# rkin100g/Nerf-Replication

Hardware: AMD Instinct MI355X
Metric: rays/sec (800x800, 64+128 samples) (higher is better)
Workload: dtype f32; 1 GPU; lego-shaped 800x800 frame = 640000 pinhole rays, 64 coarse + 128 fine hierarchical samples, 8+1-layer W=256 NeRF x2, seeded synthetic weights (latest.pth unavailable offline); BASELINE.json configs[1]; parallelism=ray-tile shard x1 (each rank generates and renders only its tile) + 1 all_gather

## Files before the change

nerf_replication_amd/_lib.py:

```python
import ctypes
import os
import subprocess

import torch

_HERE = os.path.dirname(os.path.abspath(__file__))
LIB_PATH = os.path.join(_HERE, "libnerf_mi355x.so")
CSRC = os.path.join(_HERE, "csrc")

N_SAMPLES = 64
N_IMPORTANCE = 128
PREC_F32 = 0
PREC_F16 = 1
PREC_F32X = 2
PREC_F16S = 3
PRECISIONS = {"f32": PREC_F32, "fp32": PREC_F32, "f16": PREC_F16S, "fp16": PREC_F16S, "f16s": PREC_F16S, "f16m32": PREC_F16, "f32x": PREC_F32X}


def fp32_accurate(precision_name: str) -> bool:
    return PRECISIONS[precision_name] in (PREC_F32, PREC_F32X)


_TABLE = """
nerf_abi_version  i32 :
# ... 87 lines not shown


def _protos(signatures):
    return {name: (_RETURN[ret], [_ctype(k) for k in kinds]) for name, (ret, kinds) in signatures.items()}


_PROTOS = _protos(SIGNATURES)

_TABLE_NN = """
nerf_nn_abi_version  i32 :
nerf_fused_mlp_save_floats  i64 : i64 i32 i32
nerf_fused_mlp_grad_floats  i64 : i64 i32 i32 i32
nerf_fused_mlp_forward  status : f32* i64 i32 i32 i32 i32 i32 f32*[] f32*[] f32* f32* stream
nerf_fused_mlp_backward  status : f32* f32* f32* i64 i32 i32 i32 i32 i32 f32*[] f32* f32* f32*[] f32*[] f32* stream
nerf_sh4_encode  status : f32* i64 f32* stream
nerf_field_points  status : f32* f32* f32* i64 i64 i32 i32* i64 f32[3] f32[3] f32 f32* stream
nerf_field_color_inputs  status : f32* f32* i32* i64 i64 i32 f32* f32* stream
nerf_field_color_inputs_backward  status : f32* f32* i64 f32* stream
nerf_field_raw_scatter  status : f32* f32* i32* i64 i64 f32* stream
nerf_field_raw_gather  status : f32* i32* i64 i64 f32* f32* stream
"""
NN_SIGNATURES = _parse_table(_TABLE_NN)
NN_EXPORTS = tuple(NN_SIGNATURES)
_NN_PROTOS = _protos(NN_SIGNATURES)

_TABLE_FIELD = """
nerf_field_density_seed  status : f32* i64 i64 i32 f32* stream
nerf_field_points_backward  status : f32* f32* f32* i64 i64 i32 i32* i64 f32[3] f32[3] f32 f32* f32* i32 f32* f32* f32* stream
nerf_field_sh_gradient  status : f32* i32* i64 i64 i32 f32* stream
nerf_sh4_encode_backward  status : f32* f32* i64 f32* stream
"""
FIELD_SIGNATURES = _parse_table(_TABLE_FIELD)
FIELD_EXPORTS = tuple(FIELD_SIGNATURES)
_FIELD_PROTOS = _protos(FIELD_SIGNATURES)

_TABLE_HASHGRID = """
nerf_hashgrid_deterministic_workspace_bytes  i64 : i64 i32
nerf_hashgrid_deterministic_guard_bits  i32 : i64 i32
nerf_hashgrid_backward_deterministic  status : f32* f32* i64 i32 i32 i32 i32[] f32[] f32* void* i64 stream
"""
HASHGRID_SIGNATURES = _parse_table(_TABLE_HASHGRID)
HASHGRID_EXPORTS = tuple(HASHGRID_SIGNATURES)
_HASHGRID_PROTOS = _protos(HASHGRID_SIGNATURES)

_TABLE_NN_EXACT = """
nerf_fused_mlp_exact_workspace_bytes  i64 : i32 i32 i32 i32
nerf_fused_mlp_exact_guard_bits  i32 : i64
nerf_fused_mlp_backward_exact  status : f32* f32* f32* i64 i32 i32 i32 i32 i32 f32*[] f32* f32* f32*[] f32*[] f32* void* i64 stream
"""
NN_EXACT_SIGNATURES = _parse_table(_TABLE_NN_EXACT)
NN_EXACT_EXPORTS = tuple(NN_EXACT_SIGNATURES)
_NN_EXACT_PROTOS = _protos(NN_EXACT_SIGNATURES)

_lib = None


class NerfLibraryError(RuntimeError):
    pass


def build(verbose: bool = False) -> str:
    res = subprocess.run(["make", "-C", CSRC], capture_output=True, text=True)
    if res.returncode != 0:
        raise NerfLibraryError("building libnerf_mi355x.so failed:\n" + res.stdout + res.stderr)
    if verbose:
        print(res.stdout)
    return LIB_PATH


def load():
    global _lib
    if _lib is None:
        if not os.path.exists(LIB_PATH):
            raise NerfLibraryError(
                f"{LIB_PATH} is missing: build it with `make -C {CSRC}` (or __graft_entry__.build()); "
                "there is no CPU fallback for the render path")
        lib = ctypes.CDLL(LIB_PATH)
        for name, (res, args) in (list(_PROTOS.items()) + list(_NN_PROTOS.items()) + list(_FIELD_PROTOS.items()) +
                                  list(_HASHGRID_PROTOS.items()) + list(_NN_EXACT_PROTOS.items())):
            fn = getattr(lib, name)
            fn.restype, fn.argtypes = res, args
        if lib.nerf_abi_version() != 3:
            raise NerfLibraryError("libnerf_mi355x.so ABI version mismatch")
        if lib.nerf_nn_abi_version() != 1:
            raise NerfLibraryError("libnerf_mi355x.so small-network ABI version mismatch (include/nerf_mi355x_nn.h)")
        if lib.nerf_build_flags() != 0:
            raise NerfLibraryError(f"{LIB_PATH} is a timing build (nerf_build_flags() = {lib.nerf_build_flags()}): kernels "
                                   "compiled with NERF_*_HACK_* switches compute wrong results; rebuild with `make -C csrc`")
        _lib = lib
    return _lib


class strided:

    def __init__(self, tensor):
        self.tensor = tensor


def call(name, *args):
    for table in (SIGNATURES, NN_SIGNATURES, FIELD_SIGNATURES, HASHGRID_SIGNATURES, NN_EXACT_SIGNATURES):
        if name in table:
            break
    ret, kinds = table[name]
    has_stream = kinds[-1:] == ("stream",)
    if len(args) != len(kinds) - has_stream:
        raise TypeError(f"{name} takes {len(kinds) - has_stream} arguments ({len(args)} given)")
    dev = None

    def device_pointer(t, dtype, i):
        nonlocal dev
        if t is None:
            return None
        dense = not isinstance(t, strided)
        if not dense:
            t = t.tensor
        if not t.is_cuda:
            raise NerfLibraryError(f"{name}, argument {i}: the HIP render path needs tensors on a GPU (cuda) device; got a CPU tensor")
        if (dtype is not None and t.dtype != dtype) or (dense and not t.is_contiguous()):
            raise NerfLibraryError(f"{name}, argument {i}: expected a contiguous {dtype or 'byte'} tensor, got {t.dtype} with "
                                   f"strides {tuple(t.stride())}")
        if dev is None:
            dev = t.device
        elif t.device != dev:
            raise NerfLibraryError(f"{name}, argument {i}: a tensor on {t.device}, the earlier ones on {dev}")
        return t.data_ptr()

    cargs = []
    for i, (kind, a) in enumerate(zip(kinds, args)):
        if kind in _DTYPE:
            a = device_pointer(a, _DTYPE[kind], i)
        elif kind not in _SCALAR and a is not None:
            elem, _, length = kind[:-1].partition("[")
            if length and len(a) != int(length):
                raise NerfLibraryError(f"{name}, argument {i}: a host array of {length} is needed, got {len(a)}")
            if elem in _DTYPE:
                a = (ctypes.c_void_p * len(a))(*[device_pointer(t, _DTYPE[elem], i) for t in a])
            elif not isinstance(a, ctypes.Array):
                a = (_SCALAR[elem] * len(a))(*a)
        cargs.append(a)
    fn = getattr(load(), name)
    if not has_stream:
        return fn(*cargs)
    if dev is None or dev.index == torch.cuda.current_device():
        rc = fn(*cargs, None if dev is None else torch.cuda.current_stream(dev).cuda_stream)
    else:
        with torch.cuda.device(dev):
            rc = fn(*cargs, torch.cuda.current_stream(dev).cuda_stream)
    if ret == "status":
        check(rc, name)
    return rc


def check(rc: int, what: str = ""):
# ... 38 lines not shown
```

nerf_replication_amd/csrc/nerf_kernels.hip:

```cpp
#include <hip/hip_runtime.h>
#include <cstdlib>
#include <stdio.h>
#include <string.h>
#include <math.h>
#include <utility>

#include "../../include/nerf_mi355x.h"
#include "nerf_host.h"
#include "nerf_mlp_common.h"
#include "nerf_wgrad_table.h"
#include "nerf_scan.hip.inc"
#include "nerf_mlp_f32.hip.inc"
#include "nerf_mlp_f16.hip.inc"
#include "nerf_mlp_f16s.hip.inc"
#include "nerf_mlp_f32x.hip.inc"
#include "nerf_wgrad_f32.hip.inc"
#include "nerf_mlp_bwd_f32.hip.inc"
#include "nerf_mlp_bwd_f32x.hip.inc"
#include "nerf_wgrad_bf16x3.hip.inc"
#define NERF_X_INST extern template
#include "nerf_kernels_x.inst.inc"

#include "nerf_timing_guard.h"

#include "nerf_pack.hip.inc"
#include "nerf_sampling.hip.inc"
#include "nerf_composite.hip.inc"
#include "nerf_mlp_launch.hip.inc"
#include "nerf_train_backward.hip.inc"
#include "nerf_image.hip.inc"
#include "nerf_frame.hip.inc"
#include "nerf_isosurface.hip.inc"
#include "nerf_occupancy.hip.inc"
#include "nerf_normals.hip.inc"
#include "nerf_mesh_components.hip.inc"
#include "nerf_hashgrid.hip.inc"
#include "nerf_hashgrid_det.hip.inc"
#include "nerf_fused_mlp.hip.inc"
#include "nerf_fused_mlp_exact.hip.inc"
#include "nerf_hashfield.hip.inc"

extern "C" {

int32_t nerf_abi_version(void) { return NERF_ABI_VERSION; }

int32_t nerf_build_flags(void) {
  int32_t f = 0;
#ifdef NERF_TIMING_BUILD
  f |= NERF_BUILD_TIMING;
#endif
#if NERF_ANY_TIMING_HACK || NERF_SAVE_TAPS == 0
  f |= NERF_BUILD_WRONG_NUMERICS;
#endif
  return f;
}
const char* nerf_last_error(void) { return g_err; }

}
```

nerf_replication_amd/csrc/nerf_pack.hip.inc:

```
#include "nerf_host.h"
#include "nerf_mlp_common.h"

namespace {

struct PackArgs {
  const float* p[nerf::P_COUNT];
  float* out;
};

__device__ __forceinline__ float pack_weight_elem(const PackArgs& a, long long rel, int ntiles,
                                                  int which ,
                                                  int layer) {
  using namespace nerf;
  const int q = (int)(rel & 3);
  const int lane = (int)((rel >> 2) & 63);
  const long long blk = rel >> 8;
  const int j = (int)(blk % ntiles);
  const int g = (int)(blk / ntiles);
  const int s = 4 * g + q, t = s >> 4, r = s & 15, h = lane >> 5;
  const int out = 32 * j + (lane & 31);
  switch (which) {
    case 0: { const int c = pe_xyz_feat(s, h); return c < 0 ? 0.f : a.p[P_W0][out * 63 + c]; }
    case 1: return a.p[2 * layer][out * 256 + act_feat(t, r, h)];
    case 2: { const int c = pe_xyz_feat(s, h); return c < 0 ? 0.f : a.p[10][out * 319 + c]; }
    case 3: return a.p[10][out * 319 + 63 + act_feat(t, r, h)];
    case 4: return a.p[P_WF][out * 256 + act_feat(t, r, h)];
    default: {
      if (t < 8) return a.p[P_WV][out * 283 + act_feat(t, r, h)];
      const int c = pe_dir_feat(r, h);
      return c < 0 ? 0.f : a.p[P_WV][out * 283 + 256 + c];
    }
  }
}

template <int LOG2>
__device__ __forceinline__ float act_order_value(const float* x, int rel) {
  const int h = rel >> LOG2, slot = rel & ((1 << LOG2) - 1);
  return x[nerf::act_feat(slot >> 4, slot & 15, h)];
}
__device__ __forceinline__ float pack_bias_value(const PackArgs& a, int rel) {
  const int layer = rel >> 8;
  return act_order_value<7>(layer < 8 ? a.p[2 * layer + 1] : a.p[nerf::P_BF], rel & 255);
}
__device__ __forceinline__ float pack_w_rgb_value(const float* w_rgb, int rel) {
  return act_order_value<6>(w_rgb + 128 * (rel >> 7), rel & 127);
}
__device__ __forceinline__ float pack_head_bias_value(const PackArgs& a, int rel) {
  return rel < 3 ? a.p[nerf::P_BR][rel] : a.p[nerf::P_BA][0];
}

__global__ void nerf_pack_kernel(PackArgs a) {
  using namespace nerf;
  const long long i = (long long)blockIdx.x * blockDim.x + threadIdx.x;
  if (i >= kUnfoldedFloats) return;
  constexpr long long WS = wsize(128, 8);
  float v;
  if (i < kOffL1) v = pack_weight_elem(a, i - kOffL0, 8, 0, 0);
  else if (i < kOffL5a) { const long long rel = i - kOffL1; v = pack_weight_elem(a, rel % WS, 8, 1, 1 + (int)(rel / WS)); }
  else if (i < kOffL5b) v = pack_weight_elem(a, i - kOffL5a, 8, 2, 5);
  else if (i < kOffL6) v = pack_weight_elem(a, i - kOffL5b, 8, 3, 5);
  else if (i < kOffFeat) { const long long rel = i - kOffL6; v = pack_weight_elem(a, rel % WS, 8, 1, 6 + (int)(rel / WS)); }
  else if (i < kOffViews) v = pack_weight_elem(a, i - kOffFeat, 8, 4, 0);
  else if (i < kOffBias) v = pack_weight_elem(a, i - kOffViews, 4, 5, 0);
  else if (i < kOffBiasViews) v = pack_bias_value(a, (int)(i - kOffBias));
  else if (i < kOffWAlpha) v = act_order_value<6>(a.p[P_BV], (int)(i - kOffBiasViews));
  else if (i < kOffWRgb) v = act_order_value<7>(a.p[P_WA], (int)(i - kOffWAlpha));
  else if (i < kOffHeadBias) v = pack_w_rgb_value(a.p[P_WR], (int)(i - kOffWRgb));
  else v = pack_head_bias_value(a, (int)(i - kOffHeadBias));
  a.out[i] = v;
}

constexpr int kFoldBlocks = 128 + 2 + 4 + 3;
__global__ __launch_bounds__(256) void nerf_fold_f32_kernel(const float* __restrict__ pk, float* __restrict__ fold) {
  using namespace nerf;
  __shared__ double part_sum[4][64][4];
  const int lane = threadIdx.x & 63, part = threadIdx.x >> 6, b = blockIdx.x;
  if (b >= 134) {
    constexpr int kTail4 = (int)(kFoldFloats - kFoldOffBias - 128) / 4, kGap4 = (int)(kOffFold - kUnfoldedFloats) / 4;
    static_assert(kUnfoldedFloats % 4 == 0 && kOffFold % 4 == 0 && kFoldFloats % 4 == 0 && kTail4 + kGap4 <= 3 * 256, "zero blocks");
    const int i = (b - 134) * 256 + threadIdx.x;
    const f32x4 zero = {0.f, 0.f, 0.f, 0.f};
    if (i < kTail4) reinterpret_cast<f32x4*>(fold + kFoldOffBias + 128)[i] = zero;
    else if (i < kTail4 + kGap4) reinterpret_cast<f32x4*>(fold - 4 * kGap4)[i - kTail4] = zero;
    return;
  }
  if (b >= 130) {
    const int i = (b - 130) * 256 + threadIdx.x;
    reinterpret_cast<f32x4*>(fold + kFoldOffDir)[i] = reinterpret_cast<const f32x4*>(pk + kOffViewsDir)[i];
    return;
  }
  const bool bias = b >= 128;
  int j, row, g = 0, h = 0;
  if (!bias) { j = b & 3; g = b >> 2; h = lane >> 5; row = lane & 31; }
  else {
    const int rel = (b - 128) * 64 + lane, o = act_feat((rel & 63) >> 4, rel & 15, rel >> 6);
    j = o >> 5; row = o & 31;
  }
  double acc[4] = {0.0, 0.0, 0.0, 0.0};
#pragma unroll 8
  for (int mm = 0; mm < 64; ++mm) {
    const int m = part * 64 + mm;
    const int mt = m >> 5, mh = (m >> 2) & 1, mg = 4 * mt + ((m & 31) >> 3), mq = m & 3;
    const double wv = (double)pk[kOffViews + (((long long)(mg * 4 + j) * 64 + row + 32 * mh) << 2) + mq];
    if (!bias) {
      const f32x4 wf = *reinterpret_cast<const f32x4*>(pk + kOffFeat + (((long long)(g * 8 + mt) * 64 + (m & 31) + 32 * h) << 2));
      acc[0] += wv * (double)wf.x; acc[1] += wv * (double)wf.y; acc[2] += wv * (double)wf.z; acc[3] += wv * (double)wf.w;
    } else {
      const int mr = (m & 3) + 4 * ((m & 31) >> 3);
      acc[0] += wv * (double)pk[kOffBias + 8 * 256 + mh * 128 + mt * 16 + mr];
    }
  }
#pragma unroll
  for (int q = 0; q < 4; ++q) part_sum[part][lane][q] = acc[q];
  __syncthreads();
  if (part != 0) return;
  double r[4];
#pragma unroll
  for (int q = 0; q < 4; ++q) r[q] = (part_sum[0][lane][q] + part_sum[1][lane][q]) + (part_sum[2][lane][q] + part_sum[3][lane][q]);
  if (!bias) {
// ... 150 lines not shown
  if (!pe_out) v = W[(long long)krow * ld + coff + 32 * m + irow];
  else {
    const int hp = (irow >> 2) & 1, rp = (irow & 3) + 4 * (irow >> 3);
    const int c = pe_xyz_feat(16 * m + rp, hp);
    v = c < 0 ? 0.0f : W[(long long)krow * ld + c];
  }
  store_split_f16(reinterpret_cast<_Float16*>(reinterpret_cast<char*>(a.out) + kF16ConstBytes), F, e, v);
}

template <bool SPLIT>
__global__ void nerf_pack_f16_kernel(PackArgs a) {
  using namespace nerf;
  const long long i = (long long)blockIdx.x * blockDim.x + threadIdx.x;
  constexpr long long n_const = kF16ConstBytes / 4;
  constexpr long long n_half = (long long)kF16Frags * 512;
  if (i < n_const) {
    float v = 0.0f;
    if (i < kF16OffBiasViews) v = pack_bias_value(a, (int)i);
    else if (i < kF16OffHeadBias) v = act_order_value<6>(a.p[P_BV], (int)i - kF16OffBiasViews);
    else if (i < kF16OffHeadBias + 4) v = pack_head_bias_value(a, (int)i - kF16OffHeadBias);
    a.out[i] = v;
    return;
  }
  const long long e = i - n_const;
  if (e >= n_half) return;
  const int F = (int)(e >> 9), lane = (int)((e >> 3) & 63), j = (int)(e & 7);
  const float v = frag_stream_value<Frag32x16>(a, F, lane, j);
  _Float16* out = reinterpret_cast<_Float16*>(reinterpret_cast<char*>(a.out) + kF16ConstBytes);
  if (SPLIT) store_split_f16(out, F, e, v);
  else out[e] = (_Float16)v;
}

}

extern "C" {

int64_t nerf_packed_model_bytes(int32_t precision) {
  if (precision == NERF_PREC_F32) return nerf::kPackedFloats * (int64_t)sizeof(float);
  if (precision == NERF_PREC_F16 || precision == NERF_PREC_F16S) return nerf::kF16PackedBytes + nerf::kXPackedBytes;
  if (precision == NERF_PREC_F32X) return nerf::kXPackedBytes;
  return -1;
}

static int32_t fill_pack_args(const char* entry, const float* const params[24], void* out, PackArgs& a) {
  if (!params || !out) return fail(NERF_ERR_INVALID_ARG, "%s: null argument", entry);
  for (int i = 0; i < nerf::P_COUNT; ++i) {
    if (!params[i]) return fail(NERF_ERR_INVALID_ARG, "%s: null parameter pointer", entry);
    a.p[i] = params[i];
  }
  a.out = (float*)out;
  return NERF_OK;
}

int32_t nerf_pack_model(const float* const params[24], void* packed, int32_t precision, void* stream) {
  PackArgs a;
  if (const int rc = fill_pack_args("nerf_pack_model", params, packed, a)) return rc;
  const int threads = 256;
  if (precision == NERF_PREC_F16 || precision == NERF_PREC_F32X || precision == NERF_PREC_F16S) {
    const long long n = nerf::kF16ConstBytes / 4 + (long long)nerf::kF16Frags * 512;
    const dim3 grid((unsigned)((n + threads - 1) / threads));
    hipStream_t st = (hipStream_t)stream;
    if (precision == NERF_PREC_F32X) return NERF_LAUNCH(nerf_pack_f16_kernel<true>, grid, dim3(threads), st, a);
    if (const int rc = precision == NERF_PREC_F16S ? NERF_LAUNCH(nerf_pack_f16s_kernel, grid, dim3(threads), st, a)
                                                   : NERF_LAUNCH(nerf_pack_f16_kernel<false>, grid, dim3(threads), st, a))
      return rc;
    PackArgs ax = a;
    ax.out = reinterpret_cast<float*>(reinterpret_cast<char*>(packed) + nerf::kF16PackedBytes);
    return NERF_LAUNCH(nerf_pack_f16_kernel<true>, grid, dim3(threads), st, ax);
  }
  if (precision != NERF_PREC_F32) return fail(NERF_ERR_UNSUPPORTED, "%s", "nerf_pack_model: unknown precision");
  const unsigned blocks = (unsigned)((nerf::kUnfoldedFloats + threads - 1) / threads);
  if (const int rc = NERF_LAUNCH(nerf_pack_kernel, dim3(blocks), dim3(threads), (hipStream_t)stream, a)) return rc;
  return NERF_LAUNCH(nerf_fold_f32_kernel, dim3(kFoldBlocks), dim3(256), (hipStream_t)stream, (const float*)a.out, a.out + nerf::kOffFold);
}

int64_t nerf_packed_bwd_bytes(int32_t precision) {
  if (precision == NERF_PREC_F32) return nerf::kBwdPackedFloats * (int64_t)sizeof(float);
  if (precision == NERF_PREC_F32X) return nerf::kXbPackedBytes;
  return -1;
}

int32_t nerf_pack_model_bwd(const float* const params[24], void* packed_bwd_v, int32_t precision, void* stream) {
  PackArgs a;
  if (const int rc = fill_pack_args("nerf_pack_model_bwd", params, packed_bwd_v, a)) return rc;
  if (precision == NERF_PREC_F32X) {
    const long long n = nerf::kF16ConstBytes / 4 + (long long)nerf::kXbSteps * 512;
    return NERF_LAUNCH(nerf_pack_bwd_f32x_kernel, dim3((unsigned)((n + 255) / 256)), dim3(256), (hipStream_t)stream, a);
  }
  if (precision != NERF_PREC_F32) return fail(NERF_ERR_UNSUPPORTED, "%s", "nerf_pack_model_bwd: f32 or f32x only");
  return NERF_LAUNCH(nerf_pack_bwd_kernel, dim3((unsigned)((nerf::kBwdPackedFloats + 255) / 256)), dim3(256), (hipStream_t)stream, a);
}

}
```

nerf_replication_amd/network.py:

```python
import os
import sys

import torch
import torch.nn as nn


def _sibling(name):
    import importlib
    try:
        return importlib.import_module("nerf_replication_amd." + name)
    except ModuleNotFoundError as exc:
        if exc.name != "nerf_replication_amd":
            raise
        sys.path.insert(0, os.path.dirname(os.path.dirname(os.path.abspath(__file__))))
        return importlib.import_module("nerf_replication_amd." + name)


_lib = _sibling("_lib")


def _reference_cfg():
    mod = sys.modules.get("src.config")
    return getattr(mod, "cfg", None) if mod is not None else None

# ... 6 lines not shown
            raise ValueError("the HIP kernels are built for the lego.yaml architecture: D=8, W=256, skips=[4], "
                             "xyz freq 10, dir freq 4, use_viewdirs=True")
        self.D, self.W, self.input_ch, self.input_ch_views = D, W, input_ch, input_ch_views
        self.skips, self.use_viewdirs = list(skips), True
        self.pts_linears = nn.ModuleList(
            [nn.Linear(input_ch, W)]
            + [nn.Linear(W + input_ch, W) if i in self.skips else nn.Linear(W, W) for i in range(D - 1)])
        self.views_linears = nn.ModuleList([nn.Linear(input_ch_views + W, W // 2)])
        self.feature_linear = nn.Linear(W, W)
        self.alpha_linear = nn.Linear(W, 1)
        self.rgb_linear = nn.Linear(W // 2, 3)

    def ordered_params(self):
        mods = list(self.pts_linears) + [self.views_linears[0], self.feature_linear, self.alpha_linear, self.rgb_linear]
        out = []
        for m in mods:
            out += [m.weight, m.bias]
        return out

    def forward(self, x):
        raise RuntimeError("NeRF.forward on an embedded chunk is fused into Network.forward (HIP); "
                           "call Network.forward(inputs, viewdirs, valid_mask, model)")


class Network(nn.Module):
    def __init__(self):
        super().__init__()
        cfg = _reference_cfg()
        ta = getattr(cfg, "task_arg", None) if cfg is not None else None
        self.N_samples = getattr(ta, "N_samples", 64)
        self.N_importance = getattr(ta, "N_importance", 128)
        self.chunk = getattr(ta, "chunk_size", 512)
        self.batch_size = getattr(ta, "N_rays", 1024)
        self.white_bkgd = getattr(ta, "white_bkgd", 1)
        self.use_viewdirs = bool(getattr(ta, "use_viewdirs", True))
        self.device = torch.device("cuda" if torch.cuda.is_available() else "cpu")
        self.sample_size = 64
        self.rays_size = 160000
        net = getattr(cfg, "network", None) if cfg is not None else None
        xyz_f = getattr(getattr(net, "xyz_encoder", None), "freq", 10)
        dir_f = getattr(getattr(net, "dir_encoder", None), "freq", 4)
        nerf_cfg = getattr(net, "nerf", None)
        D, W = getattr(nerf_cfg, "D", 8), getattr(nerf_cfg, "W", 256)
        skips = tuple(getattr(nerf_cfg, "skips", [4]))
        self.input_ch, self.input_ch_views = 3 + 6 * xyz_f, 3 + 6 * dir_f
        self.embed_fn = lambda x: positional_encoding(x, xyz_f)
        self.embeddirs_fn = lambda x: positional_encoding(x, dir_f)
        mk = lambda: NeRF(D=D, W=W, input_ch=self.input_ch, input_ch_views=self.input_ch_views,
                          skips=skips, use_viewdirs=self.use_viewdirs)
        self.model = mk()
        self.model_fine = mk()
        self.precision = "f32"
        self._packed = {}

    def _stream(self, model, bwd):
        tag = "fine" if model == "fine" else ""
        params = (self.model_fine if tag == "fine" else self.model).ordered_params()
        dev = params[0].device
        if dev.type != "cuda":
            raise _lib.NerfLibraryError("Network parameters are on the CPU: call .cuda() first; the render path is "
                                        "HIP-only (no CPU fallback)")
        prec = _lib.PRECISIONS[self.precision]
        if bwd:
            nbytes = int(_lib.call("nerf_packed_bwd_bytes", prec))
            if nbytes <= 0:
                raise NotImplementedError(f"the data-gradient chain runs in precision 'f32' or 'f32x', not {self.precision!r}")
            tag = "bwd" + tag
        key = (prec,) + tuple((p.data_ptr(), p._version) for p in params)
        hit = self._packed.get(tag)
        if hit is not None and hit[0] == key:
            return hit[1]
        out = torch.empty(nbytes if bwd else _lib.packed_model_bytes(prec), dtype=torch.uint8, device=dev)
        _lib.call("nerf_pack_model_bwd" if bwd else "nerf_pack_model", [p.detach().contiguous() for p in params], out, prec)
        self._packed[tag] = (key, out)
        return out

    def packed(self, model=""):
        return self._stream(model, False)

    def packed_bwd(self, model=""):
        return self._stream(model, True)

    def forward(self, inputs, viewdirs, valid_mask, model=""):
        sub = self.model_fine if model == "fine" else self.model
        if torch.is_grad_enabled() and (inputs.requires_grad or viewdirs.requires_grad or
                                        (self.training and any(p.requires_grad for p in sub.parameters()))):
            return self._forward_with_grad(inputs, viewdirs, valid_mask, model, sub)
        dev = inputs.device
        n, s = inputs.shape[0], inputs.shape[1]
        packed = self.packed(model)
        prec = _lib.PRECISIONS[self.precision]
        if valid_mask is None:
            pts = inputs.detach().to(torch.float32).contiguous()
            dirs = viewdirs.detach().to(torch.float32).contiguous()
            raw = torch.empty((n, s, 4), dtype=torch.float32, device=dev)
            _lib.call("nerf_mlp_forward", pts, dirs, n, s, packed, raw, prec)
            return raw
        flat = valid_mask.reshape(-1)
        pts = inputs.detach().reshape(-1, 3)[flat].to(torch.float32).contiguous()
        dirs = viewdirs.detach()[:, None].expand(n, s, 3).reshape(-1, 3)[flat].to(torch.float32).contiguous()
        m = pts.shape[0]
        raw_valid = torch.empty((m, 1, 4), dtype=torch.float32, device=dev)
        _lib.call("nerf_mlp_forward", pts, dirs, m, 1, packed, raw_valid, prec)
        out = torch.zeros((n * s, 4), dtype=torch.float32, device=dev)
        out[flat] = raw_valid.reshape(m, 4)
        return out.reshape(n, s, 4)

    def _forward_with_grad(self, inputs, viewdirs, valid_mask, model, sub):
        if self.precision not in ("f32", "f32x"):
            raise NotImplementedError("training runs on the fp32-accurate paths: precision 'f32' or 'f32x'")
        n, s = inputs.shape[0], inputs.shape[1]
        params = tuple(sub.ordered_params())
        if valid_mask is None:
            return _MlpFunction.apply(self, model, inputs.to(torch.float32), viewdirs.to(torch.float32), *params)
        flat = valid_mask.reshape(-1)
        pts = inputs.to(torch.float32).reshape(-1, 3)[flat][:, None, :]
        dirs = viewdirs.to(torch.float32)[:, None].expand(n, s, 3).reshape(-1, 3)[flat]
        out = torch.zeros((n * s, 4), dtype=torch.float32, device=inputs.device)
        if pts.shape[0] > 0:
            out = out.index_put((flat.nonzero(as_tuple=True)[0],), _MlpFunction.apply(self, model, pts, dirs, *params)[:, 0])
        return out.reshape(n, s, 4)
# ... 47 lines not shown
```

nerf_replication_amd/volume_renderer.py:

```python
import os
import sys

import torch


def _sibling(name):
    import importlib
    try:
        return importlib.import_module("nerf_replication_amd." + name)
    except ModuleNotFoundError as exc:
        if exc.name != "nerf_replication_amd":
            raise
        sys.path.insert(0, os.path.dirname(os.path.dirname(os.path.abspath(__file__))))
        return importlib.import_module("nerf_replication_amd." + name)


_lib = _sibling("_lib")
modes = _sibling("modes")


def _reference_cfg():
    mod = sys.modules.get("src.config")
    return getattr(mod, "cfg", None) if mod is not None else None


class Renderer:
    def __init__(self, net):
        cfg = _reference_cfg()
        self.net = net
        self.N_samples = getattr(cfg, "N_samples", 64)
        self.chunk_size = getattr(cfg, "chunk_size", 1024)
        self.white_bkgd = getattr(cfg, "white_bkgd", True)
        self.N_importance = getattr(cfg, "N_importance", 128)
        self.sample_size = 64
        self.rays_size = 160000
        self.task = getattr(cfg, "task", "test")
        self.perturb = bool(getattr(cfg, "perturb", True)) if self.task == "train" else False
        self.fast_sampling = getattr(cfg, "fast_sampling", False)
        self.weights_threshold = getattr(cfg, "weights_threshold", 0.25)
        self.t_near, self.t_far = 2.0, 6.0
        self.device = None
        self._tables = {}
        self._workspace = None
        self.occupancy = None
        self.occupancy_stats = None
        self.train_occupancy = None
        self.train_occupancy_every = 16
        self.geometry_block_rays = 4096
        if self.N_samples != _lib.N_SAMPLES or self.N_importance not in (0, _lib.N_IMPORTANCE):
            raise ValueError("HIP renderer is built for N_samples=64 and N_importance in {0,128}")

    def _get_tables(self, dev):
        tabs = self._tables.get(dev)
        if tabs is None:
            t_c = torch.linspace(self.t_near, self.t_far, self.N_samples).to(dev)
            u = torch.linspace(0.0, 1.0, steps=_lib.N_IMPORTANCE).to(dev)
            tabs = self._tables[dev] = (t_c, u)
        return tabs

    def _rand(self, shape, device):
        return torch.rand(*shape, device=device)

    def _draws(self, n, dev):
        jitter = self._rand((n, self.N_samples), dev).to(torch.float32).contiguous() if self.perturb else None
        u = None
        if self.task == "train" and self.N_importance > 0:
            u = self._rand((n, self.N_importance), dev).to(torch.float32).contiguous()
        return jitter, u

    def _get_workspace(self, nbytes, dev):
        ws = self._workspace
        if ws is None or ws.device != dev or ws.numel() < nbytes:
            self._workspace = None
            ws = self._workspace = torch.empty(nbytes, dtype=torch.uint8, device=dev)
        return ws

    def _scheduled_grid(self):
        grid = self.train_occupancy
        if grid.stale(self.net, "fine") and grid.uses >= self.train_occupancy_every:
            grid.refresh(self.net, models=("fine",))
        grid.uses += 1
        return grid

    def render(self, batch):
        rays_o, rays_d = batch["rays_o"], batch["rays_d"]
        self.device = dev = rays_o.device
        if dev.type != "cuda":
            raise _lib.NerfLibraryError("Renderer.render needs rays on a GPU: the render path is HIP-only")
        B, N, _ = rays_o.shape
        n = B * N
        rays_grad = torch.is_grad_enabled() and (rays_o.requires_grad or rays_d.requires_grad)
        if not rays_grad:
            rays_o, rays_d = rays_o.detach(), rays_d.detach()
        o = rays_o.reshape(n, 3).to(torch.float32).contiguous()
        d = rays_d.reshape(n, 3).to(torch.float32).contiguous()
        facts = modes.facts(self, modes.RENDER, rays_grad, n)
        path = modes.resolve(facts, self, dev)
        grid = self._scheduled_grid() if facts.with_grad and facts.train_occupancy else None
        draws = self._draws(n, dev) if facts.stochastic else ()
        return self._RENDER[path](self, facts, o, d, draws, grid)

    def _empty(self, facts, o, d, draws, grid):
        if facts.with_grad:
            return torch.empty((0, 3), device=o.device), torch.empty((0,), device=o.device)
        return self._frame_arguments(facts, o, d)[-2:]

    def _step(self, facts, o, d, draws, grid):
        kw = {} if grid is None else {"occupancy": grid}
        return _sibling("training").render_with_grad(self, o, d, *draws, **kw)

    def _frame_arguments(self, facts, o, d):
        n, dev = o.shape[0], o.device
        t_c, u = self._get_tables(dev)
        pk_c = self.net.packed("")
        pk_f = self.net.packed("fine") if self.N_importance > 0 else None
        rgb = torch.empty((n, 3), dtype=torch.float32, device=dev)
        depth = torch.empty((n,), dtype=torch.float32, device=dev)
        fast = int(bool(self.fast_sampling) and self.N_importance > 0)
        modes_ = (int(self.N_importance), int(bool(self.white_bkgd)), _lib.PRECISIONS[facts.precision], fast, float(self.weights_threshold))
        return (o, d, n, pk_c, pk_f, t_c, u), modes_, fast, rgb, depth

    def _frame(self, facts, o, d, draws, grid):
        head, modes_, fast, rgb, depth = self._frame_arguments(facts, o, d)
        ws = self._get_workspace(int(_lib.call("nerf_render_workspace_bytes", head[2], self.N_importance, fast)), o.device)
        _lib.call("nerf_render_forward", *head, *modes_, ws, ws.numel(), rgb, depth)
        return rgb, depth

    def _frame_stochastic(self, facts, o, d, draws, grid):
        head, modes_, _, rgb, depth = self._frame_arguments(facts, o, d)
        ws = self._get_workspace(int(_lib.call("nerf_render_stochastic_workspace_bytes", head[2], self.N_importance)), o.device)
        _lib.call("nerf_render_forward_stochastic", *head, *draws, *modes_, ws, ws.numel(), rgb, depth)
        return rgb, depth

    def _frame_occupancy(self, facts, o, d, draws, grid):
        head, modes_, fast, rgb, depth = self._frame_arguments(facts, o, d)
        n, occ = head[2], self.occupancy
        occ_c, occ_f = occ.bits[""], occ.bits["fine"] if self.N_importance > 0 else None
        ws = self._get_workspace(int(_lib.call("nerf_render_occupancy_workspace_bytes", n, self.N_importance, fast)), o.device)
        evaluated = torch.empty(2, dtype=torch.int64, device=o.device) if self.occupancy_stats is not None else None
        _lib.call("nerf_render_forward_occupancy", *head, *modes_, occ_c, occ_f, *occ.lookup_args(), evaluated, ws, ws.numel(),
                  rgb, depth)
        if evaluated is not None:
            self.occupancy_stats.append((evaluated.clone(), (_lib.N_SAMPLES * n, (_lib.N_SAMPLES + _lib.N_IMPORTANCE) * n)))
        return rgb, depth

    _RENDER = {"empty": _empty, "frame": _frame, "frame_stochastic": _frame_stochastic, "frame_occupancy": _frame_occupancy,
               "step": _step, "step_masked": _step, "step_coarse": _step, "step_culled": _step}

    def render_geometry(self, batch):
        rays_o, rays_d = batch["rays_o"], batch["rays_d"]
        self.device = dev = rays_o.device
        if dev.type != "cuda":
            raise _lib.NerfLibraryError("Renderer.render_geometry needs rays on a GPU: the render path is HIP-only")
        B, N, _ = rays_o.shape
        n = B * N
        facts = modes.facts(self, modes.GEOMETRY, rays_o.requires_grad or rays_d.requires_grad, n)
        path = modes.resolve(facts, self, dev)
        block = self.geometry_block_rays
        o = rays_o.detach().reshape(n, 3).to(torch.float32).contiguous()
        d = rays_d.detach().reshape(n, 3).to(torch.float32).contiguous()
        new = lambda *shape: torch.empty(shape, dtype=torch.float32, device=dev)
        out = {"rgb": new(n, 3), "depth": new(n), "acc": new(n), "normal": new(n, 3)}
        if path == "empty":
            return out
        prec = _lib.PRECISIONS[facts.precision]
        t_c, u = self._get_tables(dev)
        fine = self.N_importance > 0
        model = "fine" if fine else ""
        pk_c = self.net.packed("")
        pk = self.net.packed(model)
        pk_b = self.net.packed_bwd(model)
        S_c, S = _lib.N_SAMPLES, _lib.N_SAMPLES + (_lib.N_IMPORTANCE if fine else 0)
        nb_max = min(block, n)
        raw_c = new(nb_max, S_c, 4)
        t_sorted, raw_f = (new(nb_max, S), new(nb_max, S, 4)) if fine else (None, None)
        grad = new(nb_max, S, 3)
        ws = torch.empty(int(_lib.call("nerf_density_gradient_point_bytes")) * ((nb_max * S + 31) // 32 * 32), dtype=torch.uint8, device=dev)
        white = int(bool(self.white_bkgd))
        for r0 in range(0, n, block):
            nb = min(block, n - r0)
            ob, db = o[r0:r0 + nb], d[r0:r0 + nb]
            if fine:
                _lib.call("nerf_mlp_forward_rays_density", ob, db, t_c, 0, nb, S_c, pk_c, raw_c, prec)
                _lib.call("nerf_sample_fine", raw_c, t_c, u, nb, t_sorted, None, None, 0.0, 0.0)
                _lib.call("nerf_mlp_forward_rays_for_compositing", ob, db, t_sorted, S, nb, S, pk, raw_f, prec)
                raw, tv, stride = raw_f, t_sorted, S
            else:
                _lib.call("nerf_mlp_forward_rays", ob, db, t_c, 0, nb, S_c, pk_c, raw_c, prec)
                raw, tv, stride = raw_c, t_c, 0
            _lib.call("nerf_composite", raw, tv, stride, nb, S, white, out["rgb"][r0:r0 + nb], out["depth"][r0:r0 + nb], None)
            _lib.call("nerf_density_gradient", ob, db, tv, stride, nb, S, pk, pk_b, 1, None, grad, prec, ws, ws.numel())
            _lib.call("nerf_composite_normals", raw, tv, stride, nb, S, grad, out["normal"][r0:r0 + nb], out["acc"][r0:r0 + nb])
        return out
```

Before: 638,800 rays/s.

## Permute hidden units by co-inactivity to pair dead ReLUs for tile skipping

Adds a calibration pass that renders a few sample rays and counts how often pairs of hidden units are both inactive, per layer. A greedy matching then pairs units that tend to be zero together, and the f32 weights are repacked in that permuted order. The likely aim is to let the existing masked MLP kernels skip more zero tiles. Calibration runs automatically on the second large render with unchanged weights. It adds a host sync, a device-to-host copy and a CPU matching step once per weight version.

```diff
diff --git a/include/nerf_mi355x_order.h b/include/nerf_mi355x_order.h
--- /dev/null
+++ b/include/nerf_mi355x_order.h
@@ -0,0 +1,19 @@
+#ifndef NERF_MI355X_ORDER_H
+#define NERF_MI355X_ORDER_H
+
+#include "nerf_mi355x.h"
+
+#ifdef __cplusplus
+extern "C" {
+#endif
+
+int32_t nerf_pack_model_ordered(const float* const params[24], const uint8_t* order, void* packed, int32_t precision, void* stream);
+
+int32_t nerf_unit_order_stats(const float* save, int64_t n_points, int32_t* counts, void* stream);
+
+int32_t nerf_unit_order_match(const int32_t counts[65536], int32_t order[256]);
+
+#ifdef __cplusplus
+}
+#endif
+#endif
diff --git a/nerf_replication_amd/_lib.py b/nerf_replication_amd/_lib.py
--- a/nerf_replication_amd/_lib.py
+++ b/nerf_replication_amd/_lib.py
@@ -163,6 +163,15 @@
 NN_EXACT_EXPORTS = tuple(NN_EXACT_SIGNATURES)
 _NN_EXACT_PROTOS = _protos(NN_EXACT_SIGNATURES)
 
+_TABLE_ORDER = """
+nerf_pack_model_ordered  status : f32*[24] u8* void* i32 stream
+nerf_unit_order_stats  status : f32* i64 i32* stream
+nerf_unit_order_match  i32 : i32[65536] i32[256]
+"""
+ORDER_SIGNATURES = _parse_table(_TABLE_ORDER)
+ORDER_EXPORTS = tuple(ORDER_SIGNATURES)
+_ORDER_PROTOS = _protos(ORDER_SIGNATURES)
+
 _lib = None
 
 
@@ -188,7 +197,7 @@
                 "there is no CPU fallback for the render path")
         lib = ctypes.CDLL(LIB_PATH)
         for name, (res, args) in (list(_PROTOS.items()) + list(_NN_PROTOS.items()) + list(_FIELD_PROTOS.items()) +
-                                  list(_HASHGRID_PROTOS.items()) + list(_NN_EXACT_PROTOS.items())):
+                                  list(_HASHGRID_PROTOS.items()) + list(_NN_EXACT_PROTOS.items()) + list(_ORDER_PROTOS.items())):
             fn = getattr(lib, name)
             fn.restype, fn.argtypes = res, args
         if lib.nerf_abi_version() != 3:
@@ -209,7 +218,7 @@
 
 
 def call(name, *args):
-    for table in (SIGNATURES, NN_SIGNATURES, FIELD_SIGNATURES, HASHGRID_SIGNATURES, NN_EXACT_SIGNATURES):
+    for table in (SIGNATURES, NN_SIGNATURES, FIELD_SIGNATURES, HASHGRID_SIGNATURES, NN_EXACT_SIGNATURES, ORDER_SIGNATURES):
         if name in table:
             break
     ret, kinds = table[name]
diff --git a/nerf_replication_amd/csrc/nerf_kernels.hip b/nerf_replication_amd/csrc/nerf_kernels.hip
--- a/nerf_replication_amd/csrc/nerf_kernels.hip
+++ b/nerf_replication_amd/csrc/nerf_kernels.hip
@@ -24,6 +24,7 @@
 #include "nerf_timing_guard.h"
 
 #include "nerf_pack.hip.inc"
+#include "nerf_unit_order.hip.inc"
 #include "nerf_sampling.hip.inc"
 #include "nerf_composite.hip.inc"
 #include "nerf_mlp_launch.hip.inc"
diff --git a/nerf_replication_amd/csrc/nerf_pack.hip.inc b/nerf_replication_amd/csrc/nerf_pack.hip.inc
--- a/nerf_replication_amd/csrc/nerf_pack.hip.inc
+++ b/nerf_replication_amd/csrc/nerf_pack.hip.inc
@@ -1,3 +1,4 @@
+#include "../../include/nerf_mi355x_order.h"
 #include "nerf_host.h"
 #include "nerf_mlp_common.h"
 
@@ -8,9 +9,13 @@
   float* out;
 };
 
+__device__ __forceinline__ int ordered_unit(const uint8_t* order, int l, int position) {
+  return order ? (int)order[l * nerf::kHidden + position] : position;
+}
+
 __device__ __forceinline__ float pack_weight_elem(const PackArgs& a, long long rel, int ntiles,
                                                   int which ,
-                                                  int layer) {
+                                                  int layer, const uint8_t* order) {
   using namespace nerf;
   const int q = (int)(rel & 3);
   const int lane = (int)((rel >> 2) & 63);
@@ -20,11 +25,11 @@
   const int s = 4 * g + q, t = s >> 4, r = s & 15, h = lane >> 5;
   const int out = 32 * j + (lane & 31);
   switch (which) {
-    case 0: { const int c = pe_xyz_feat(s, h); return c < 0 ? 0.f : a.p[P_W0][out * 63 + c]; }
-    case 1: return a.p[2 * layer][out * 256 + act_feat(t, r, h)];
-    case 2: { const int c = pe_xyz_feat(s, h); return c < 0 ? 0.f : a.p[10][out * 319 + c]; }
-    case 3: return a.p[10][out * 319 + 63 + act_feat(t, r, h)];
-    case 4: return a.p[P_WF][out * 256 + act_feat(t, r, h)];
+    case 0: { const int c = pe_xyz_feat(s, h); return c < 0 ? 0.f : a.p[P_W0][ordered_unit(order, 0, out) * 63 + c]; }
+    case 1: return a.p[2 * layer][ordered_unit(order, layer, out) * 256 + ordered_unit(order, layer - 1, act_feat(t, r, h))];
+    case 2: { const int c = pe_xyz_feat(s, h); return c < 0 ? 0.f : a.p[10][ordered_unit(order, 5, out) * 319 + c]; }
+    case 3: return a.p[10][ordered_unit(order, 5, out) * 319 + 63 + ordered_unit(order, 4, act_feat(t, r, h))];
+    case 4: return a.p[P_WF][out * 256 + ordered_unit(order, 7, act_feat(t, r, h))];
     default: {
       if (t < 8) return a.p[P_WV][out * 283 + act_feat(t, r, h)];
       const int c = pe_dir_feat(r, h);
@@ -38,10 +43,19 @@
   const int h = rel >> LOG2, slot = rel & ((1 << LOG2) - 1);
   return x[nerf::act_feat(slot >> 4, slot & 15, h)];
 }
+template <int LOG2>
+__device__ __forceinline__ float act_order_value_ordered(const float* x, int rel, const uint8_t* order, int l) {
+  const int h = rel >> LOG2, slot = rel & ((1 << LOG2) - 1);
+  return x[ordered_unit(order, l, nerf::act_feat(slot >> 4, slot & 15, h))];
+}
 __device__ __forceinline__ float pack_bias_value(const PackArgs& a, int rel) {
   const int layer = rel >> 8;
   return act_order_value<7>(layer < 8 ? a.p[2 * layer + 1] : a.p[nerf::P_BF], rel & 255);
 }
+__device__ __forceinline__ float pack_bias_value_ordered(const PackArgs& a, int rel, const uint8_t* order) {
+  const int layer = rel >> 8;
+  return layer < 8 ? act_order_value_ordered<7>(a.p[2 * layer + 1], rel & 255, order, layer) : act_order_value<7>(a.p[nerf::P_BF], rel & 255);
+}
 __device__ __forceinline__ float pack_w_rgb_value(const float* w_rgb, int rel) {
   return act_order_value<6>(w_rgb + 128 * (rel >> 7), rel & 127);
 }
@@ -49,22 +63,22 @@
   return rel < 3 ? a.p[nerf::P_BR][rel] : a.p[nerf::P_BA][0];
 }
 
-__global__ void nerf_pack_kernel(PackArgs a) {
+__global__ void nerf_pack_kernel(PackArgs a, const uint8_t* __restrict__ order) {
   using namespace nerf;
   const long long i = (long long)blockIdx.x * blockDim.x + threadIdx.x;
   if (i >= kUnfoldedFloats) return;
   constexpr long long WS = wsize(128, 8);
   float v;
-  if (i < kOffL1) v = pack_weight_elem(a, i - kOffL0, 8, 0, 0);
-  else if (i < kOffL5a) { const long long rel = i - kOffL1; v = pack_weight_elem(a, rel % WS, 8, 1, 1 + (int)(rel / WS)); }
-  else if (i < kOffL5b) v = pack_weight_elem(a, i - kOffL5a, 8, 2, 5);
-  else if (i < kOffL6) v = pack_weight_elem(a, i - kOffL5b, 8, 3, 5);
-  else if (i < kOffFeat) { const long long rel = i - kOffL6; v = pack_weight_elem(a, rel % WS, 8, 1, 6 + (int)(rel / WS)); }
-  else if (i < kOffViews) v = pack_weight_elem(a, i - kOffFeat, 8, 4, 0);
-  else if (i < kOffBias) v = pack_weight_elem(a, i - kOffViews, 4, 5, 0);
-  else if (i < kOffBiasViews) v = pack_bias_value(a, (int)(i - kOffBias));
+  if (i < kOffL1) v = pack_weight_elem(a, i - kOffL0, 8, 0, 0, order);
+  else if (i < kOffL5a) { const long long rel = i - kOffL1; v = pack_weight_elem(a, rel % WS, 8, 1, 1 + (int)(rel / WS), order); }
+  else if (i < kOffL5b) v = pack_weight_elem(a, i - kOffL5a, 8, 2, 5, order);
+  else if (i < kOffL6) v = pack_weight_elem(a, i - kOffL5b, 8, 3, 5, order);
+  else if (i < kOffFeat) { const long long rel = i - kOffL6; v = pack_weight_elem(a, rel % WS, 8, 1, 6 + (int)(rel / WS), order); }
+  else if (i < kOffViews) v = pack_weight_elem(a, i - kOffFeat, 8, 4, 0, order);
+  else if (i < kOffBias) v = pack_weight_elem(a, i - kOffViews, 4, 5, 0, order);
+  else if (i < kOffBiasViews) v = pack_bias_value_ordered(a, (int)(i - kOffBias), order);
   else if (i < kOffWAlpha) v = act_order_value<6>(a.p[P_BV], (int)(i - kOffBiasViews));
-  else if (i < kOffWRgb) v = act_order_value<7>(a.p[P_WA], (int)(i - kOffWAlpha));
+  else if (i < kOffWRgb) v = act_order_value_ordered<7>(a.p[P_WA], (int)(i - kOffWAlpha), order, 7);
   else if (i < kOffHeadBias) v = pack_w_rgb_value(a.p[P_WR], (int)(i - kOffWRgb));
   else v = pack_head_bias_value(a, (int)(i - kOffHeadBias));
   a.out[i] = v;
@@ -321,6 +335,12 @@
   return NERF_OK;
 }
 
+static int32_t pack_f32(const PackArgs& a, const uint8_t* order, hipStream_t st) {
+  const unsigned blocks = (unsigned)((nerf::kUnfoldedFloats + 255) / 256);
+  if (const int rc = NERF_LAUNCH(nerf_pack_kernel, dim3(blocks), dim3(256), st, a, order)) return rc;
+  return NERF_LAUNCH(nerf_fold_f32_kernel, dim3(kFoldBlocks), dim3(256), st, (const float*)a.out, a.out + nerf::kOffFold);
+}
+
 int32_t nerf_pack_model(const float* const params[24], void* packed, int32_t precision, void* stream) {
   PackArgs a;
   if (const int rc = fill_pack_args("nerf_pack_model", params, packed, a)) return rc;
@@ -338,9 +358,14 @@
     return NERF_LAUNCH(nerf_pack_f16_kernel<true>, grid, dim3(threads), st, ax);
   }
   if (precision != NERF_PREC_F32) return fail(NERF_ERR_UNSUPPORTED, "%s", "nerf_pack_model: unknown precision");
-  const unsigned blocks = (unsigned)((nerf::kUnfoldedFloats + threads - 1) / threads);
-  if (const int rc = NERF_LAUNCH(nerf_pack_kernel, dim3(blocks), dim3(threads), (hipStream_t)stream, a)) return rc;
-  return NERF_LAUNCH(nerf_fold_f32_kernel, dim3(kFoldBlocks), dim3(256), (hipStream_t)stream, (const float*)a.out, a.out + nerf::kOffFold);
+  return pack_f32(a, nullptr, (hipStream_t)stream);
+}
+
+int32_t nerf_pack_model_ordered(const float* const params[24], const uint8_t* order, void* packed, int32_t precision, void* stream) {
+  PackArgs a;
+  if (const int rc = fill_pack_args("nerf_pack_model_ordered", params, packed, a)) return rc;
+  if (precision != NERF_PREC_F32) return fail(NERF_ERR_UNSUPPORTED, "%s", "nerf_pack_model_ordered: f32 only");
+  return pack_f32(a, order, (hipStream_t)stream);
 }
 
 int64_t nerf_packed_bwd_bytes(int32_t precision) {
diff --git a/nerf_replication_amd/csrc/nerf_unit_order.hip.inc b/nerf_replication_amd/csrc/nerf_unit_order.hip.inc
--- /dev/null
+++ b/nerf_replication_amd/csrc/nerf_unit_order.hip.inc
@@ -0,0 +1,67 @@
+#include "../../include/nerf_mi355x_order.h"
+#include "nerf_host.h"
+#include "nerf_mlp_common.h"
+#include "nerf_unit_order_match.h"
+
+namespace {
+
+__global__ __launch_bounds__(256) void nerf_unit_order_stats_kernel(const float* __restrict__ save, long long n_points,
+                                                                    int32_t* __restrict__ counts) {
+  using namespace nerf;
+  const int rb = blockIdx.x, layer = blockIdx.y, j = threadIdx.x, lane = j & 63, wave = j >> 6;
+  const long long n_tiles = TrainSave::pad32(n_points) / kTilePts;
+  const u32x4* bits = reinterpret_cast<const u32x4*>(save + TrainSave::off_bits(n_points));
+  __shared__ unsigned on[4][2][4];
+  const int jt = j >> 5, jh = (j >> 2) & 1, jr = (j & 3) + 4 * ((j & 31) >> 3);
+  int32_t cnt[32];
+#pragma unroll
+  for (int i = 0; i < 32; ++i) cnt[i] = 0;
+  for (long long t0 = 0; t0 < n_tiles; t0 += 4) {
+    const long long tile = t0 + wave;
+    u32x4 m = {~0u, ~0u, ~0u, ~0u};
+    if (tile < n_tiles) m = bits[(tile * TrainSave::kMasked + layer) * 64 + lane];
+#pragma unroll
+    for (int d = 16; d >= 1; d >>= 1) {
+      m.x |= __shfl_xor(m.x, d); m.y |= __shfl_xor(m.y, d); m.z |= __shfl_xor(m.z, d); m.w |= __shfl_xor(m.w, d);
+    }
+    if ((lane & 31) == 0) {
+      unsigned* dst = on[wave][lane >> 5];
+      dst[0] = m.x; dst[1] = m.y; dst[2] = m.z; dst[3] = m.w;
+    }
+    __syncthreads();
+#pragma unroll
+    for (int w = 0; w < 4; ++w) {
+      const bool off_j = ((on[w][jh][jt >> 1] >> (16 * (jt & 1) + jr)) & 1u) == 0u;
+      const unsigned off0 = ~on[w][0][rb >> 1] >> (16 * (rb & 1)), off1 = ~on[w][1][rb >> 1] >> (16 * (rb & 1));
+      if (off_j) {
+#pragma unroll
+        for (int i = 0; i < 32; ++i) {
+          const int r = (i & 3) + 4 * (i >> 3);
+          cnt[i] += (int32_t)((((i >> 2) & 1 ? off1 : off0) >> r) & 1u);
+        }
+      }
+    }
+    __syncthreads();
+  }
+#pragma unroll
+  for (int i = 0; i < 32; ++i) counts[((long long)layer * kHidden + 32 * rb + i) * kHidden + j] = cnt[i];
+}
+
+}
+
+extern "C" {
+
+int32_t nerf_unit_order_stats(const float* save, int64_t n_points, int32_t* counts, void* stream) {
+  if (n_points < 1 || n_points > 0x7fffffffLL * 32) return fail(NERF_ERR_INVALID_ARG, "%s", "nerf_unit_order_stats: bad size");
+  if (!save || !counts) return fail(NERF_ERR_INVALID_ARG, "%s", "nerf_unit_order_stats: null argument");
+  if (((uintptr_t)save & 15) != 0) return fail(NERF_ERR_INVALID_ARG, "%s", "nerf_unit_order_stats: save must be 16-byte aligned");
+  return NERF_LAUNCH(nerf_unit_order_stats_kernel, dim3(8, 8), dim3(256), (hipStream_t)stream, save, (long long)n_points, counts);
+}
+
+int32_t nerf_unit_order_match(const int32_t counts[65536], int32_t order[256]) {
+  if (!counts || !order) return fail(NERF_ERR_INVALID_ARG, "%s", "nerf_unit_order_match: null argument");
+  nerf::unit_order_match(counts, order);
+  return NERF_OK;
+}
+
+}
diff --git a/nerf_replication_amd/csrc/nerf_unit_order_match.h b/nerf_replication_amd/csrc/nerf_unit_order_match.h
--- /dev/null
+++ b/nerf_replication_amd/csrc/nerf_unit_order_match.h
@@ -0,0 +1,48 @@
+#pragma once
+#include <stdint.h>
+
+#include <algorithm>
+#include <vector>
+
+#include "nerf_layout.h"
+
+namespace nerf {
+
+inline void unit_order_match(const int32_t* counts, int32_t* order) {
+  constexpr int N = kHidden;
+  constexpr int kPairs = N * (N - 1) / 2;
+  struct Pair { int32_t c; int16_t i, j; };
+  int64_t lo = counts[1], hi = counts[1];
+  for (int i = 0; i < N; ++i)
+    for (int j = i + 1; j < N; ++j) { lo = std::min<int64_t>(lo, counts[i * N + j]); hi = std::max<int64_t>(hi, counts[i * N + j]); }
+  std::vector<Pair> pairs(kPairs);
+  if (hi - lo < (1 << 16)) {
+    std::vector<int32_t> start(hi - lo + 2, 0);
+    for (int i = 0; i < N; ++i)
+      for (int j = i + 1; j < N; ++j) ++start[hi - counts[i * N + j] + 1];
+    for (size_t k = 1; k < start.size(); ++k) start[k] += start[k - 1];
+    for (int i = 0; i < N; ++i)
+      for (int j = i + 1; j < N; ++j) pairs[start[hi - counts[i * N + j]]++] = Pair{counts[i * N + j], (int16_t)i, (int16_t)j};
+  } else {
+    int n = 0;
+    for (int i = 0; i < N; ++i)
+      for (int j = i + 1; j < N; ++j) pairs[n++] = Pair{counts[i * N + j], (int16_t)i, (int16_t)j};
+    std::stable_sort(pairs.begin(), pairs.end(), [](const Pair& a, const Pair& b) { return a.c > b.c; });
+  }
+  bool taken[N] = {};
+  std::vector<Pair> chosen;
+  chosen.reserve(N / 2);
+  for (const Pair& p : pairs) {
+    if (taken[p.i] || taken[p.j]) continue;
+    taken[p.i] = taken[p.j] = true;
+    chosen.push_back(p);
+    if ((int)chosen.size() == N / 2) break;
+  }
+  std::sort(chosen.begin(), chosen.end(), [](const Pair& a, const Pair& b) { return a.c != b.c ? a.c > b.c : a.i < b.i; });
+  for (int s = 0; s < N / 2; ++s) {
+    order[act_feat(s >> 4, s & 15, 0)] = chosen[s].i;
+    order[act_feat(s >> 4, s & 15, 1)] = chosen[s].j;
+  }
+}
+
+}
diff --git a/nerf_replication_amd/network.py b/nerf_replication_amd/network.py
--- a/nerf_replication_amd/network.py
+++ b/nerf_replication_amd/network.py
@@ -82,21 +82,61 @@
         self.model_fine = mk()
         self.precision = "f32"
         self._packed = {}
-
-    def _stream(self, model, bwd):
+        self._orders = {}
+        self._large_renders = {}
+
+    def _stream_key(self, model):
         tag = "fine" if model == "fine" else ""
         params = (self.model_fine if tag == "fine" else self.model).ordered_params()
-        dev = params[0].device
-        if dev.type != "cuda":
+        if params[0].device.type != "cuda":
             raise _lib.NerfLibraryError("Network parameters are on the CPU: call .cuda() first; the render path is "
                                         "HIP-only (no CPU fallback)")
+        return tag, params, (_lib.PRECISIONS[self.precision],) + tuple((p.data_ptr(), p._version) for p in params)
+
+    def unit_order(self, model=""):
+        tag, _, key = self._stream_key(model)
+        hit = self._orders.get(tag)
+        return hit[1] if hit is not None and hit[0] == key else None
+
+    def rendered_before(self, model=""):
+        tag, _, key = self._stream_key(model)
+        seen = self._large_renders.get(tag) == key
+        self._large_renders[tag] = key
+        return seen
+
+    def set_unit_order(self, model, order):
+        tag, params, key = self._stream_key(model)
+        self._packed.pop("inf" + tag, None)
+        if order is None:
+            self._orders.pop(tag, None)
+            return
+        host = torch.as_tensor(order).detach().cpu().to(torch.int64)
+        if host.shape != (8, 256) or not bool((host.sort(dim=1).values == torch.arange(256)).all()):
+            raise ValueError("a unit order is [8, 256] with every row a permutation of 0..255")
+        self._orders[tag] = (key, host.to(torch.uint8).contiguous().to(params[0].device))
+
+    def packed_inference(self, model=""):
+        order = self.unit_order(model) if _lib.PRECISIONS[self.precision] == _lib.PREC_F32 else None
+        if order is None:
+            return self.packed(model)
+        tag, params, key = self._stream_key(model)
+        hit = self._packed.get("inf" + tag)
+        if hit is not None and hit[0] == key and hit[2] is order:
+            return hit[1]
+        out = torch.empty(_lib.packed_model_bytes(_lib.PREC_F32), dtype=torch.uint8, device=params[0].device)
+        _lib.call("nerf_pack_model_ordered", [p.detach().contiguous() for p in params], order, out, _lib.PREC_F32)
+        self._packed["inf" + tag] = (key, out, order)
+        return out
+
+    def _stream(self, model, bwd):
+        tag, params, key = self._stream_key(model)
+        dev = params[0].device
         prec = _lib.PRECISIONS[self.precision]
         if bwd:
             nbytes = int(_lib.call("nerf_packed_bwd_bytes", prec))
             if nbytes <= 0:
                 raise NotImplementedError(f"the data-gradient chain runs in precision 'f32' or 'f32x', not {self.precision!r}")
             tag = "bwd" + tag
-        key = (prec,) + tuple((p.data_ptr(), p._version) for p in params)
         hit = self._packed.get(tag)
         if hit is not None and hit[0] == key:
             return hit[1]
diff --git a/nerf_replication_amd/volume_renderer.py b/nerf_replication_amd/volume_renderer.py
--- a/nerf_replication_amd/volume_renderer.py
+++ b/nerf_replication_amd/volume_renderer.py
@@ -22,6 +22,10 @@
 def _reference_cfg():
     mod = sys.modules.get("src.config")
     return getattr(mod, "cfg", None) if mod is not None else None
+
+
+UNIT_ORDER_SAMPLE_RAYS = 16
+UNIT_ORDER_MIN_RAYS = 160000
 
 
 class Renderer:
@@ -47,6 +51,8 @@
         self.train_occupancy = None
         self.train_occupancy_every = 16
         self.geometry_block_rays = 4096
+        self.unit_order = "auto"
+        self.unit_order_min_rays = UNIT_ORDER_MIN_RAYS
         if self.N_samples != _lib.N_SAMPLES or self.N_importance not in (0, _lib.N_IMPORTANCE):
             raise ValueError("HIP renderer is built for N_samples=64 and N_importance in {0,128}")
 
@@ -109,11 +115,79 @@
         kw = {} if grid is None else {"occupancy": grid}
         return _sibling("training").render_with_grad(self, o, d, *draws, **kw)
 
+    def _unit_order_on(self):
+        if self.unit_order not in ("auto", "off"):
+            raise ValueError(f"Renderer.unit_order must be 'auto' or 'off', got {self.unit_order!r}")
+        return (self.unit_order == "auto" and os.environ.get("NERF_UNIT_ORDER") != "0"
+                and _lib.PRECISIONS[modes.precision_of(self.net)] == _lib.PREC_F32)
+
+    def _models(self):
+        return ("", "fine") if self.N_importance > 0 else ("",)
+
+    def _inference_streams(self, o=None, d=None):
+        if not self._unit_order_on():
+            return self.net.packed(""), self.net.packed("fine") if self.N_importance > 0 else None
+        if (o is not None and o.shape[0] >= self.unit_order_min_rays and not torch.cuda.is_current_stream_capturing()
+                and any(self.net.unit_order(m) is None for m in self._models())
+                and all([self.net.rendered_before(m) for m in self._models()])):
+            self._calibrate(o, d)
+        return self.net.packed_inference(""), self.net.packed_inference("fine") if self.N_importance > 0 else None
+
+    def calibrate_unit_order(self, batch):
+        if modes.precision_of(self.net) not in ("f32", "fp32"):
+            raise NotImplementedError("unit orders exist for precision 'f32' only")
+        if torch.cuda.is_current_stream_capturing():
+            raise RuntimeError("calibrate_unit_order synchronises: not during a graph capture")
+        rays_o, rays_d = batch["rays_o"], batch["rays_d"]
+        o = rays_o.detach().reshape(-1, 3).to(torch.float32).contiguous()
+        d = rays_d.detach().reshape(-1, 3).to(torch.float32).contiguous()
+        if o.shape[0] == 0:
+            raise ValueError("calibrate_unit_order needs at least one ray")
+        return self._calibrate(o, d)
+
+    def _calibrate(self, o, d):
+        import ctypes
+        n, dev = o.shape[0], o.device
+        k = UNIT_ORDER_SAMPLE_RAYS
+        os_, ds_ = torch.empty((k, 3), dtype=torch.float32, device=dev), torch.empty((k, 3), dtype=torch.float32, device=dev)
+        for i in range(k):
+            r = (2 * i + 1) * n // (2 * k)
+            os_[i].copy_(o[r])
+            ds_[i].copy_(d[r])
+        t_c, u = self._get_tables(dev)
+        prec = _lib.PREC_F32
+        new = lambda *shape: torch.empty(shape, dtype=torch.float32, device=dev)
+        S_c, S = _lib.N_SAMPLES, _lib.N_SAMPLES + _lib.N_IMPORTANCE
+        counts = {}
+        raw_c, save = new(k, S_c, 4), new(int(_lib.call("nerf_train_save_floats", k * S_c)))
+        _lib.call("nerf_mlp_forward_rays_save", os_, ds_, t_c, 0, k, S_c, self.net.packed(""), raw_c, save, prec)
+        counts[""] = torch.empty((8, 256, 256), dtype=torch.int32, device=dev)
+        _lib.call("nerf_unit_order_stats", save, k * S_c, counts[""])
+        if self.N_importance > 0:
+            t_sorted, raw_f = new(k, S), new(k, S, 4)
+            _lib.call("nerf_sample_fine", raw_c, t_c, u, k, t_sorted, None, None, 0.0, 0.0)
+            save = None
+            save = new(int(_lib.call("nerf_train_save_floats", k * S)))
+            _lib.call("nerf_mlp_forward_rays_save", os_, ds_, t_sorted, S, k, S, self.net.packed("fine"), raw_f, save, prec)
+            counts["fine"] = torch.empty((8, 256, 256), dtype=torch.int32, device=dev)
+            _lib.call("nerf_unit_order_stats", save, k * S, counts["fine"])
+        orders = {}
+        for model, c in counts.items():
+            host = c.cpu().numpy()
+            order = torch.empty((8, 256), dtype=torch.int32)
+            for l in range(8):
+                out = (ctypes.c_int32 * 256)()
+                _lib.check(_lib.call("nerf_unit_order_match", (ctypes.c_int32 * 65536).from_buffer(host[l]), out),
+                           "nerf_unit_order_match")
+                order[l] = torch.tensor(list(out), dtype=torch.int32)
+            self.net.set_unit_order(model, order)
+            orders[model] = self.net.unit_order(model)
+        return orders
+
     def _frame_arguments(self, facts, o, d):
         n, dev = o.shape[0], o.device
         t_c, u = self._get_tables(dev)
-        pk_c = self.net.packed("")
-        pk_f = self.net.packed("fine") if self.N_importance > 0 else None
+        pk_c, pk_f = self._inference_streams(o, d)
         rgb = torch.empty((n, 3), dtype=torch.float32, device=dev)
         depth = torch.empty((n,), dtype=torch.float32, device=dev)
         fast = int(bool(self.fast_sampling) and self.N_importance > 0)
@@ -167,7 +241,8 @@
         t_c, u = self._get_tables(dev)
         fine = self.N_importance > 0
         model = "fine" if fine else ""
-        pk_c = self.net.packed("")
+        pk_c, pk_fwd = self._inference_streams()
+        pk_fwd = pk_fwd if fine else pk_c
         pk = self.net.packed(model)
         pk_b = self.net.packed_bwd(model)
         S_c, S = _lib.N_SAMPLES, _lib.N_SAMPLES + (_lib.N_IMPORTANCE if fine else 0)
@@ -183,7 +258,7 @@
             if fine:
                 _lib.call("nerf_mlp_forward_rays_density", ob, db, t_c, 0, nb, S_c, pk_c, raw_c, prec)
                 _lib.call("nerf_sample_fine", raw_c, t_c, u, nb, t_sorted, None, None, 0.0, 0.0)
-                _lib.call("nerf_mlp_forward_rays_for_compositing", ob, db, t_sorted, S, nb, S, pk, raw_f, prec)
+                _lib.call("nerf_mlp_forward_rays_for_compositing", ob, db, t_sorted, S, nb, S, pk_fwd, raw_f, prec)
                 raw, tv, stride = raw_f, t_sorted, S
             else:
                 _lib.call("nerf_mlp_forward_rays", ob, db, t_c, 0, nb, S_c, pk_c, raw_c, prec)
```

Result: faster. 722,300 rays/s (median of 6 runs) (+13.1%).
